# faircloth-lab/tapir

Hardware: AMD Instinct MI355X
Metric: alignment columns/sec (site-rate+PI) (higher is better)
Workload: dtype f64

## Files before the change

tapir_amd/csrc/pi_kernels.hpp:

```cpp
#pragma once
#include <hip/hip_runtime.h>
#include <cstdint>
#include "gtr_model.hpp"
#include "tree_program.hpp"
#include "quadpack_device.hpp"
#include "site_rate_params.hpp"
#include "pi_rate.hpp"
#include "tphip.h"

namespace tphip {

constexpr int kTimeTile = 16;
constexpr int kIvTile = 8;

struct ClassifyParams {
    const uint8_t* states;
    int64_t ncols_total;
    int32_t ntaxa;
    const LocusModel* models;
    const int64_t* locus_offsets;
    const int32_t* chunk_locus;
    const int32_t* chunk_index;
    double* rate;
    double* subst;
// ... 465 lines not shown
        }
        if ((bal[it] >> lane) & 1ull) {
            const int32_t col = (int32_t)(base + it * kCompactChunkBlock + threadIdx.x);
            const int before = woff + __popcll(bal[it] & below);
            if (kClasses) {
                const int erank = weoff + __popcll(bal_easy[it] & below);
                const int res = reserved_before(erank, reserve_q);
                const bool easy = (bal_easy[it] >> lane) & 1ull;
                if (easy && reserved_before((int64_t)erank + 1, reserve_q) != res) work_cols[lo + n_main + res] = col;
                else work_cols[lo + before - res] = col;
            } else {
                work_cols[lo + before] = col;
            }
        }
    }
}

__device__ __forceinline__ double wave_sum(double v) {
#pragma unroll
    for (int o = 32; o > 0; o >>= 1) v += __shfl_xor(v, o);
    return v;
}

__global__ __launch_bounds__(kPiBlock) void pi_partial_kernel(PiParams P) {
    __shared__ double red[kTimeTile][4];
    __shared__ double tile[kTimeTile][16 * 17];
    const int chunk = blockIdx.x;
    const int locus = P.chunk_locus[chunk];
    const int64_t lo = P.locus_offsets[locus], hi = P.locus_offsets[locus + 1];
    const int64_t base = lo + (int64_t)P.chunk_index[chunk] * kPiChunk;
    const int lane = threadIdx.x & 63, wave = threadIdx.x >> 6;
    double r[kPiColsPerThread];
    bool ok[kPiColsPerThread];
#pragma unroll
    for (int j = 0; j < kPiColsPerThread; ++j) {
        const int64_t col = base + j * kPiBlock + threadIdx.x;
        r[j] = (col < hi) ? finalize_rate(P, col) : __longlong_as_double(0x7ff8000000000000ll);
        ok[j] = isfinite(r[j]) && r[j] != 0.0;
    }
    {
        __shared__ double packed_rate[kPiChunk];
        __shared__ int wave_count[kPiBlock / 64];
        int c = 0;
#pragma unroll
        for (int j = 0; j < kPiColsPerThread; ++j) c += ok[j] ? 1 : 0;
        int inc = c;
#pragma unroll
        for (int o = 1; o < 64; o <<= 1) {
            const int up = __shfl_up(inc, o);
            if (lane >= o) inc += up;
        }
        if (lane == 63) wave_count[wave] = inc;
        __syncthreads();
        int pos = inc - c, total = 0;
#pragma unroll
        for (int w = 0; w < kPiBlock / 64; ++w) { pos += (w < wave) ? wave_count[w] : 0; total += wave_count[w]; }
#pragma unroll
        for (int j = 0; j < kPiColsPerThread; ++j) if (ok[j]) packed_rate[pos++] = r[j];
        __syncthreads();
#pragma unroll
        for (int j = 0; j < kPiColsPerThread; ++j) {
            const int idx = j * kPiBlock + (int)threadIdx.x;
            ok[j] = idx < total;
            r[j] = ok[j] ? packed_rate[idx] : __longlong_as_double(0x7ff8000000000000ll);
        }
    }
    const int Wp = P.T + 2 * P.n_i;
    double* out = P.partial + (size_t)chunk * Wp;
    for (int t0 = 0; t0 < P.T; t0 += kTimeTile) {
        double acc[kTimeTile];
#pragma unroll
        for (int i = 0; i < kTimeTile; ++i) acc[i] = 0.0;
#pragma unroll
        for (int j = 0; j < kPiColsPerThread; ++j) {
            if (!ok[j]) continue;
            const double c = 16.0 * (r[j] * r[j]);
            const double q = exp(-(4.0 * r[j]));
            double p = exp(-(4.0 * r[j] * (double)t0));
#pragma unroll
            for (int i = 0; i < kTimeTile; ++i) {
                acc[i] = fma(c * (double)(t0 + i), p, acc[i]);
                p *= q;
            }
        }
        {
            const int slot = (threadIdx.x >> 4) * 17 + (threadIdx.x & 15);
#pragma unroll
            for (int i = 0; i < kTimeTile; ++i) tile[i][slot] = acc[i];
        }
        __syncthreads();
        {
            const int i = threadIdx.x >> 4, seg = threadIdx.x & 15;
            const double* src = &tile[i][seg * 17];
            double sum = 0.0;
#pragma unroll
            for (int k = 0; k < 16; ++k) sum += src[k];
            sum += __shfl_xor(sum, 8);
            sum += __shfl_xor(sum, 4);
            sum += __shfl_xor(sum, 2);
            sum += __shfl_xor(sum, 1);
            if (seg == 0 && t0 + i < P.T) out[t0 + i] = sum;
        }
        __syncthreads();
    }
    for (int k0 = 0; k0 < P.n_i; k0 += kIvTile) {
        double si[kIvTile], se[kIvTile];
#pragma unroll
        for (int kk = 0; kk < kIvTile; ++kk) { si[kk] = 0.0; se[kk] = 0.0; }
#pragma unroll 1
        for (int j = 0; j < kPiColsPerThread; ++j) {
            if (!ok[j]) continue;
            GkFactors F;
            double have_h = -1.0;
#pragma unroll
            for (int kk = 0; kk < kIvTile; ++kk) {
                const int k = k0 + kk;
                if (k < P.n_i) {
                    const double a = (double)P.intervals[2 * k], b = (double)P.intervals[2 * k + 1];
                    double res, err = 0.0;
                    if (P.integ_mode == TPHIP_INTEG_QUADPACK) {
                        const double hl = 0.5 * (b - a);
                        if (4.0 * r[j] * hl < 30.0) {
                            if (hl != have_h) { gk_factors(r[j], hl, F); have_h = hl; }
                            quad_townsend_factored(a, b, r[j], F, res, err);
                        } else {
                            quad_townsend<false>(a, b, r[j], nullptr, res, err);
                        }
                    } else {
                        res = integral_closed(a, b, r[j]);
                    }
                    si[kk] += res;
                    se[kk] += err;
                }
            }
        }
#pragma unroll
        for (int kk = 0; kk < kIvTile; ++kk) {
            const int k = k0 + kk;
            if (k < P.n_i) {
                const double s1 = wave_sum(si[kk]), s2 = wave_sum(se[kk]);
                if (lane == 0) { red[2 * kk][wave] = s1; red[2 * kk + 1][wave] = s2; }
            }
        }
        __syncthreads();
        if (threadIdx.x < 2 * kIvTile && k0 + (int)(threadIdx.x >> 1) < P.n_i) {
            const int kk = threadIdx.x >> 1, which = threadIdx.x & 1;
            out[P.T + which * P.n_i + k0 + kk] =
                ((red[threadIdx.x][0] + red[threadIdx.x][1]) + red[threadIdx.x][2]) + red[threadIdx.x][3];
        }
        __syncthreads();
    }
}

constexpr int kPiReduceBlock = 64;
__global__ __launch_bounds__(kPiReduceBlock) void pi_reduce_kernel(const double* __restrict__ partial, const int64_t* __restrict__ locus_chunk_offsets,
                                 int32_t T, const int32_t* __restrict__ times, int32_t n_t, int32_t n_i,
                                 double* __restrict__ tables) {
    const int locus = blockIdx.x;
    const int64_t c0 = locus_chunk_offsets[locus], c1 = locus_chunk_offsets[locus + 1];
    const int Wp = T + 2 * n_i, W = T + n_t + 2 * n_i;
    double* row = tables + (size_t)locus * W;
    for (int w = threadIdx.x; w < Wp + n_t; w += blockDim.x) {
        const int src = (w < Wp) ? w : times[w - Wp];
        double s = 0.0;
        int64_t c = c0;
        for (; c + 8 <= c1; c += 8) {
            double v[8];
#pragma unroll
            for (int u = 0; u < 8; ++u) v[u] = partial[(size_t)(c + u) * Wp + src];
#pragma unroll
            for (int u = 0; u < 8; ++u) s += v[u];
        }
        for (; c < c1; ++c) s += partial[(size_t)c * Wp + src];
        const int dst = (w < T) ? w : (w < Wp ? w + n_t : T + (w - Wp));
        row[dst] = s;
    }
}

__global__ void corrected_rates_kernel(PiParams P, int64_t n, double* __restrict__ out) {
    const int64_t i = (int64_t)blockIdx.x * blockDim.x + threadIdx.x;
    if (i < n) out[i] = finalize_rate(P, i);
}

__global__ void townsend_dense_kernel(const double* __restrict__ rates, int64_t n, const double* __restrict__ times,
                                      int32_t n_times, double* __restrict__ out) {
    const int64_t i = (int64_t)blockIdx.x * blockDim.x + threadIdx.x;
    if (i >= n) return;
    const double r = rates[i];
    for (int k = 0; k < n_times; ++k) out[(size_t)k * n + i] = townsend_pi<false>(times[k], r, nullptr);
}

__global__ void quad_sites_kernel(const double* __restrict__ rates, int64_t n, double a, double b, int32_t integ_mode,
                                  double* __restrict__ integral, double* __restrict__ abserr) {
    const int64_t i = (int64_t)blockIdx.x * blockDim.x + threadIdx.x;
    if (i >= n) return;
    const double r = rates[i];
    double res = __longlong_as_double(0x7ff8000000000000ll), err = res;
    if (isfinite(r)) {
        err = 0.0;
        if (integ_mode == TPHIP_INTEG_QUADPACK) quad_townsend<false>(a, b, r, nullptr, res, err);
        else res = integral_closed(a, b, r);
    }
    integral[i] = res;
    abserr[i] = err;
}

__global__ __launch_bounds__(256) void state_histogram_kernel(const uint8_t* __restrict__ states, int64_t ncols_total,
                                                              int32_t ntaxa, const int64_t* __restrict__ locus_offsets,
                                                              unsigned long long* __restrict__ hist) {
    __shared__ unsigned int h[16];
    const int locus = blockIdx.x;
    const int64_t lo = locus_offsets[locus], hi = locus_offsets[locus + 1];
    if (threadIdx.x < 16) h[threadIdx.x] = 0;
    __syncthreads();
    unsigned int mine[16];
#pragma unroll
    for (int m = 0; m < 16; ++m) mine[m] = 0;
    for (int t = 0; t < ntaxa; ++t) {
        const uint8_t* row = states + (int64_t)t * ncols_total;
        for (int64_t c = lo + threadIdx.x; c < hi; c += blockDim.x) {
            unsigned m = row[c] & 15u;
            m = m ? m : 15u;
#pragma unroll
            for (int k = 0; k < 16; ++k) mine[k] += (m == (unsigned)k);
        }
    }
#pragma unroll
    for (int m = 0; m < 16; ++m) {
        unsigned v = mine[m];
        for (int o = 32; o > 0; o >>= 1) v += __shfl_xor(v, o);
        if ((threadIdx.x & 63) == 0) atomicAdd(&h[m], v);
    }
    __syncthreads();
    if (threadIdx.x < 16) hist[(size_t)locus * 16 + threadIdx.x] = h[threadIdx.x];
}

}
```

tapir_amd/csrc/site_launch_plan.hpp:

```cpp
#pragma once
#include <algorithm>
#include <cmath>
#include <cstddef>
#include <cstdint>
#include <cstdio>
#include <cstdlib>
#include <cstring>
#include <optional>
#include <utility>
#include <vector>

#include "launch_constants.hpp"
#include "tphip.h"

namespace tphip {

inline size_t site_lds_bytes(int depth) { return (kSiteLdsHeader + (size_t)depth * 12 * kSiteBlock) * sizeof(double); }
inline size_t mixed_lds_bytes(int depth) { return (kMixedLdsHeader + (size_t)depth * 12 * kSiteBlock) * sizeof(double); }

struct PlanKnobs {
    std::optional<long> site_chunk, site_waves, site_grid_mult;
    std::optional<char> site_spill, site_persistent, site_mixed, site_tail_order, site_share_work, compact_chunked, dedup;
    std::optional<double> site_first_fraction, site_reserve;
    std::optional<std::pair<double, double>> site_class_weights;
    std::optional<int> host_split;
};

constexpr const char* kPlanKnobNames[] = {
    "TPHIP_SITE_CHUNK", "TPHIP_SITE_SPILL", "TPHIP_SITE_PERSISTENT", "TPHIP_SITE_MIXED", "TPHIP_SITE_WAVES",
    "TPHIP_SITE_FIRST_FRACTION", "TPHIP_SITE_GRID_MULT", "TPHIP_SITE_TAIL_ORDER", "TPHIP_SITE_SHARE_WORK", "TPHIP_SITE_RESERVE",
    "TPHIP_SITE_CLASS_WEIGHTS", "TPHIP_COMPACT_CHUNKED", "TPHIP_DEDUP", "TPHIP_HOST_SPLIT"};

inline bool set_plan_knob(PlanKnobs* k, const char* name, const char* text) {
    const auto is = [name](const char* n) { return strcmp(name, n) == 0; };
    if (is("TPHIP_SITE_CHUNK")) k->site_chunk = atol(text);
    else if (is("TPHIP_SITE_SPILL")) k->site_spill = text[0];
    else if (is("TPHIP_SITE_PERSISTENT")) k->site_persistent = text[0];
    else if (is("TPHIP_SITE_MIXED")) k->site_mixed = text[0];
    else if (is("TPHIP_SITE_WAVES")) k->site_waves = atol(text);
    else if (is("TPHIP_SITE_FIRST_FRACTION")) k->site_first_fraction = atof(text);
    else if (is("TPHIP_SITE_GRID_MULT")) k->site_grid_mult = atol(text);
    else if (is("TPHIP_SITE_TAIL_ORDER")) k->site_tail_order = text[0];
    else if (is("TPHIP_SITE_SHARE_WORK")) k->site_share_work = text[0];
    else if (is("TPHIP_SITE_RESERVE")) k->site_reserve = atof(text);
    else if (is("TPHIP_SITE_CLASS_WEIGHTS")) {
        double a = 0, b = 0;
        if (sscanf(text, "%lf,%lf", &a, &b) == 2) k->site_class_weights = std::make_pair(a, b);
    }
    else if (is("TPHIP_COMPACT_CHUNKED")) k->compact_chunked = text[0];
    else if (is("TPHIP_DEDUP")) k->dedup = text[0];
    else if (is("TPHIP_HOST_SPLIT")) k->host_split = atoi(text);
    else return false;
    return true;
}

struct SiteShape {
    int64_t ncols = 0, nloci = 0, max_locus_cols = 0;
    int32_t ntaxa = 0;
    int32_t nwords = 0;
    int32_t stack_depth = 0;
    int32_t model = 0;
    int32_t ncat = 0;
    int32_t start_rule = 0;
    int32_t pattern_dedup = 0;
    int32_t T = 0, n_i = 0;
};

struct SiteLaunch {
    int32_t start_rule = 0;
    int32_t dedup_mode = 0;
    int32_t chunk_cols = kSiteBlock;
    int32_t waves = 0;
    int32_t persistent = 1;
    int32_t mixed_few_waves = 0;
    int64_t mixed_switch_cols = 0;
    int32_t mixed = 0;
    int32_t grid_mult = 1;
    int32_t lds_depth = 0;
    double first_fraction = 0.0;
    int32_t tail_order = 1;
    int32_t share_work = 0, reserve_q = 0, w_slow = 0, w_easy = 0;
    int32_t compact_chunked = 0;
};

inline int64_t site_grid(const SiteLaunch& s, int64_t n_site_chunks) {
    return s.mixed ? s.waves : s.persistent ? (int64_t)s.waves * s.grid_mult : n_site_chunks;
}

inline int32_t site_chunk_cols(const PlanKnobs& knobs) {
    int64_t cc = 512;
    if (knobs.site_chunk && *knobs.site_chunk >= kSiteBlock) cc = *knobs.site_chunk;
    return (int32_t)cc;
}

template <typename Occupancy>
SiteLaunch decide_site_launch(const SiteShape& shape, int num_cus, const PlanKnobs& knobs, Occupancy&& occupancy) {
    SiteLaunch s;
    const int64_t ncols = shape.ncols;
    const int nwords = shape.nwords, stack_depth = shape.stack_depth;
    s.start_rule = shape.start_rule == TPHIP_START_AUTO
                       ? ((shape.ntaxa >= kFirstStepMinTaxa || shape.ncat > 1) ? TPHIP_START_PARSIMONY : TPHIP_START_REFERENCE)
                       : shape.start_rule;
    s.chunk_cols = site_chunk_cols(knobs);
    int per_cu = occupancy(nwords <= 2 ? 2 : nwords <= 8 ? 8 : kStreamWords, site_lds_bytes(stack_depth));
    if (per_cu < 1) per_cu = 1;
    s.waves = per_cu * num_cus;
    s.lds_depth = stack_depth;
    {
        const int keep = (int)((160 * 1024 / 8 - kSiteLdsHeader * sizeof(double)) / (12 * kSiteBlock * sizeof(double)));
        bool want = nwords > 8 && stack_depth > keep && per_cu < 8;
        if (knobs.site_spill) want = (*knobs.site_spill == '1') && nwords > 8 && stack_depth > 1;
        if (want) {
            const int depth = std::max(1, std::min(keep, stack_depth - 1));
            const int per2 = occupancy(kStreamWordsSpill, site_lds_bytes(depth));
            if (per2 > per_cu && ncols / ((int64_t)per2 * num_cus) >= 1000) {
                s.lds_depth = depth;
                s.waves = per2 * num_cus;
            }
        }
    }
    s.persistent = (ncols / s.waves >= 1000) ? 1 : 0;
    if (knobs.site_persistent) s.persistent = (*knobs.site_persistent == '1');
    if (!s.persistent && s.lds_depth < stack_depth) {
        s.lds_depth = stack_depth;
        s.waves = per_cu * num_cus;
    }
    const bool mixed_fits = nwords <= 8 && ncols < ((int64_t)1 << kMixedColBits);
    s.mixed = (!s.persistent && mixed_fits) ? 1 : 0;
    if (knobs.site_mixed) s.mixed = (*knobs.site_mixed == '1') && mixed_fits;
    if (s.mixed) {
        int per3 = 0;
        const size_t lds3 = mixed_lds_bytes(stack_depth);
        const int64_t simds = 4 * (int64_t)num_cus;
        const double est_rounds = (double)ncols * (s.start_rule == TPHIP_START_REFERENCE ? 2.2 : 1.4) / (double)(kSiteBlock * simds);
        if (lds3 > 160 * 1024 || (per3 = occupancy(kMixedVariant + (nwords <= 2 ? 2 : 8), lds3)) < 1) s.mixed = 0;
        else if (est_rounds >= 28.0 && per3 < 8 && !knobs.site_mixed) s.mixed = 0;
        else {
            s.persistent = 0;
            const int64_t want = (per3 < 8) ? std::min<int64_t>(simds, (int64_t)per3 * num_cus) : 8 * (int64_t)num_cus;
            s.mixed_few_waves = (int32_t)std::min<int64_t>(simds, want);
            s.mixed_switch_cols = (int64_t)(24.0 * (double)(kSiteBlock * simds) / (s.start_rule == TPHIP_START_REFERENCE ? 3.7 : 2.4));
            s.waves = (int32_t)std::max<int64_t>(1, std::min<int64_t>(want, (ncols + kSiteBlock - 1) / kSiteBlock));
        }
    }
    if (knobs.site_waves && *knobs.site_waves >= 1) { s.waves = (int32_t)*knobs.site_waves; s.mixed_switch_cols = 0; }
    {
        const int64_t share = ncols / std::max(1, s.waves);
        const bool uneven = s.persistent && share >= 1500;
        s.grid_mult = uneven ? 3 : 1;
        const int64_t avg_locus = ncols / std::max<int64_t>(1, shape.nloci);
        s.first_fraction = !uneven ? 0.0 : (share >= 2 * avg_locus ? 0.9 : 0.8);
        if (uneven && s.lds_depth < stack_depth) s.first_fraction = 0.8;
        if (knobs.site_first_fraction) s.first_fraction = *knobs.site_first_fraction;
        if (knobs.site_grid_mult && *knobs.site_grid_mult >= 1 && *knobs.site_grid_mult <= 16) s.grid_mult = (int32_t)*knobs.site_grid_mult;
        if (knobs.site_tail_order) s.tail_order = (*knobs.site_tail_order != '0');
        double reserve = kDefaultReserve, w_slow = 2.9, w_easy = 2.04;
        s.share_work = (uneven && share < 2 * avg_locus) ? 1 : 0;
        if (knobs.site_share_work) s.share_work = (*knobs.site_share_work != '0');
        if (knobs.site_reserve) reserve = *knobs.site_reserve;
        if (knobs.site_class_weights) {
            const double a = knobs.site_class_weights->first, b = knobs.site_class_weights->second;
            if (a > 0 && b > 0 && a <= 16 && b <= 16) { w_slow = a; w_easy = b; }
        }
        if (!s.persistent || s.mixed || shape.max_locus_cols > ((int64_t)1 << 24)) s.share_work = 0;
        s.w_slow = std::max<int32_t>(1, (int32_t)lround(w_slow * (1 << kShareWeightShift)));
        s.w_easy = std::max<int32_t>(1, (int32_t)lround(w_easy * (1 << kShareWeightShift)));
        reserve = (s.share_work && s.grid_mult > 1) ? std::min(std::max(reserve, 0.0), 1.0) : 0.0;
        s.reserve_q = (int32_t)lround(reserve * (1 << kReserveShift));
    }
    s.compact_chunked = shape.max_locus_cols > 2048 ? 1 : 0;
    if (knobs.compact_chunked) s.compact_chunked = (*knobs.compact_chunked != '0');
    s.dedup_mode = shape.pattern_dedup;
    if (knobs.dedup)
        s.dedup_mode = (*knobs.dedup == '0') ? DEDUP_OFF : (*knobs.dedup == '1') ? DEDUP_ON : DEDUP_AUTO;
    if (s.dedup_mode == DEDUP_AUTO && ncols < kDedupAutoMinColumns) s.dedup_mode = DEDUP_OFF;
    return s;
}

inline int32_t host_split_groups(const PlanKnobs& knobs) {
    return knobs.host_split ? std::max(1, std::min(64, *knobs.host_split)) : 2;
}

struct ChunkTables {
    std::vector<int32_t> site_chunk_locus, site_chunk_index, pi_chunk_locus, pi_chunk_index;
    std::vector<int64_t> locus_pichunk_offsets;
};

inline ChunkTables build_chunk_tables(const int64_t* locus_offsets, int64_t nloci, int32_t chunk_cols) {
    ChunkTables t;
    t.locus_pichunk_offsets.assign((size_t)nloci + 1, 0);
    for (int64_t l = 0; l < nloci; ++l) {
        const int64_t S = locus_offsets[l + 1] - locus_offsets[l];
        const int64_t ns_max = std::max<int64_t>(1, (S + chunk_cols / 2) / chunk_cols);
        for (int64_t c = 0; c < ns_max && S > 0; ++c) { t.site_chunk_locus.push_back((int32_t)l); t.site_chunk_index.push_back((int32_t)c); }
        for (int64_t c = 0; c * kPiChunk < S; ++c) { t.pi_chunk_locus.push_back((int32_t)l); t.pi_chunk_index.push_back((int32_t)c); }
        t.locus_pichunk_offsets[l + 1] = (int64_t)t.pi_chunk_locus.size();
    }
    return t;
}

struct WorkspaceLayout {
    size_t work_cols = 0, work_cols2 = 0, work_count = 0, work_prefix = 0, slice_prefix = 0;
    size_t work_class = 0, work_wprefix = 0, part_prefix = 0, part_start = 0;
    size_t chunk_cnt = 0;
    size_t partial = 0, packed = 0;
    size_t hash = 0, dup_of = 0, tab_key = 0, tab_val = 0, dedup_on = 0;
    size_t spill = 0;
    size_t total = 0;
};

inline WorkspaceLayout layout_workspace(const SiteShape& shape, const SiteLaunch& s, int64_t n_pi_chunks) {
    WorkspaceLayout w;
    size_t off = 0;
    const auto take = [&off](size_t bytes) { const size_t at = off; off = (off + bytes + 255) / 256 * 256; return at; };
    const size_t ncols = (size_t)shape.ncols, nloci = (size_t)shape.nloci;
    w.work_cols = take(sizeof(int32_t) * ncols);
    if (!s.persistent || s.reserve_q > 0) w.work_cols2 = take(sizeof(int32_t) * ncols);
    w.work_count = take(sizeof(int32_t) * nloci);
    w.work_prefix = take(sizeof(int64_t) * (nloci + 1));
    w.slice_prefix = take(sizeof(int64_t) * (nloci + 1));
    w.work_class = take(sizeof(int32_t) * 2 * nloci);
    w.work_wprefix = take(sizeof(int64_t) * (nloci + 1));
    w.part_prefix = take(sizeof(int64_t) * 2 * (nloci + 1));
    w.part_start = take(sizeof(int64_t) * 2 * (nloci + 1));
    w.chunk_cnt = take(sizeof(int32_t) * 2 * (size_t)std::max<int64_t>(1, n_pi_chunks));
    w.partial = take(sizeof(double) * (size_t)n_pi_chunks * (size_t)(shape.T + 2 * shape.n_i));
    w.packed = take(sizeof(uint32_t) * (size_t)shape.nwords * ncols);
    if (s.dedup_mode != DEDUP_OFF) {
        w.hash = take(sizeof(uint64_t) * ncols);
        w.dup_of = take(sizeof(int32_t) * ncols);
        w.tab_key = take(sizeof(unsigned long long) * 2 * ncols);
        w.tab_val = take(sizeof(int32_t) * 2 * ncols);
        w.dedup_on = take(sizeof(int32_t) * nloci);
    }
    if (s.lds_depth < shape.stack_depth) {
        const size_t rows = (size_t)s.waves * (size_t)s.grid_mult * (size_t)(shape.stack_depth - s.lds_depth);
        w.spill = take(rows * 12 * kSiteBlock * sizeof(double));
    }
    w.total = off + 256;
    return w;
}

}
```

tapir_amd/csrc/tphip.hip:

```cpp
#include <hip/hip_runtime.h>

#include <algorithm>
#include <cmath>
#include <cstddef>
#include <cstdio>
#include <cstdlib>
#include <cstring>
#include <string>
#include <vector>

#include "gtr_model.hpp"
#include "gtr_setup_kernel.hpp"
#include "locus_lik_params.hpp"
#include "locus_value_params.hpp"
#include "pattern_kernels.hpp"
#include <hipcub/hipcub.hpp>
#include "pi_kernels.hpp"
#include "site_rate_params.hpp"
#include "tphip.h"
#include "tree_program.hpp"
#include "tphip_internal.hpp"

using namespace tphip;

// ... 561 lines not shown
    ClassifyParams C;
    C.states = d_states; C.ncols_total = p->ncols; C.ntaxa = p->ntaxa; C.models = p->d_models.p;
    C.locus_offsets = p->d_offsets.p; C.chunk_locus = p->d_pi_chunk_locus.p; C.chunk_index = p->d_pi_chunk_index.p;
    C.rate = d_rate; C.subst = d_subst; C.lnl = d_lnl; C.flag = d_flag; C.nres = d_nres;
    C.chrono_length = p->prog.chrono_length;
    C.steps = (const int2*)p->d_cls_steps.p; C.tail_pops = p->prog.cls_tail_pops; C.max_pops = p->prog.cls_max_pops;
    C.packed = (uint32_t*)((char*)ws + p->ws.packed);
    C.start_scale = (p->site.start_rule == TPHIP_START_REFERENCE) ? 0.0 : 1.0;
    const bool dedup = p->site.dedup_mode != DEDUP_OFF && p->n_pi_chunks > 0;
    C.hash = dedup ? (uint64_t*)((char*)ws + p->ws.hash) : nullptr;
    DedupParams D;
    if (dedup) {
        D.locus_offsets = p->d_offsets.p; D.chunk_locus = p->d_pi_chunk_locus.p; D.chunk_index = p->d_pi_chunk_index.p;
        D.hash = C.hash; D.packed = C.packed; D.nwords = p->nwords; D.ncols_total = p->ncols; D.flag = d_flag;
        D.dup_of = (int32_t*)((char*)ws + p->ws.dup_of);
        D.tab_key = (unsigned long long*)((char*)ws + p->ws.tab_key); D.tab_val = (int32_t*)((char*)ws + p->ws.tab_val);
        D.on = (int32_t*)((char*)ws + p->ws.dedup_on); D.mode = p->site.dedup_mode;
        D.rate = d_rate; D.subst = d_subst; D.lnl = d_lnl;
    }
    if (p->n_pi_chunks > 0) {
        classify_kernel<<<dim3((unsigned)p->n_pi_chunks), dim3(kPiBlock), 0, st>>>(C);
        if (dedup) {
            if (p->max_locus_cols > 2048) dedup_estimate_kernel<1024><<<dim3((unsigned)p->nloci), dim3(1024), 0, st>>>(D);
            else dedup_estimate_kernel<256><<<dim3((unsigned)p->nloci), dim3(256), 0, st>>>(D);
            dedup_insert_kernel<<<dim3((unsigned)p->n_pi_chunks), dim3(256), 0, st>>>(D);
            dedup_resolve_kernel<<<dim3((unsigned)p->n_pi_chunks), dim3(256), 0, st>>>(D);
        }
        if (p->site.share_work) {
            int32_t* work_class = (int32_t*)((char*)ws + p->ws.work_class);
            if (p->site.compact_chunked) {
                launch_compact_chunked(p, d_flag, d_lnl, work_cols, work_count, work_class, ws, st);
            } else {
                int32_t* scratch = p->site.reserve_q > 0 ? (int32_t*)((char*)ws + p->ws.work_cols2) : nullptr;
                if (p->max_locus_cols > 2048) compact_classes_kernel<1024><<<dim3((unsigned)p->nloci), dim3(1024), 0, st>>>(d_flag, p->d_offsets.p, work_cols, work_count, d_lnl, p->site.reserve_q, scratch, work_class);
                else compact_classes_kernel<256><<<dim3((unsigned)p->nloci), dim3(256), 0, st>>>(d_flag, p->d_offsets.p, work_cols, work_count, d_lnl, p->site.reserve_q, scratch, work_class);
            }
            ScanClasses SC;
            SC.cls = work_class; SC.reserve_q = p->site.reserve_q; SC.w_slow = p->site.w_slow; SC.w_easy = p->site.w_easy;
            SC.locus_offsets = p->d_offsets.p;
            SC.wprefix = (int64_t*)((char*)ws + p->ws.work_wprefix); SC.part_prefix = (int64_t*)((char*)ws + p->ws.part_prefix);
            SC.part_start = (int64_t*)((char*)ws + p->ws.part_start);
            HIP_TRY(launch_scan_counts_kernel(st, work_count, p->nloci, p->site.chunk_cols, (int64_t*)((char*)ws + p->ws.work_prefix),
                                              (int64_t*)((char*)ws + p->ws.slice_prefix), &SC));
        } else {
            if (p->site.compact_chunked) launch_compact_chunked(p, d_flag, nullptr, work_cols, work_count, nullptr, ws, st);
            else if (p->max_locus_cols > 2048) compact_kernel<1024><<<dim3((unsigned)p->nloci), dim3(1024), 0, st>>>(d_flag, p->d_offsets.p, work_cols, work_count);
            else compact_kernel<256><<<dim3((unsigned)p->nloci), dim3(256), 0, st>>>(d_flag, p->d_offsets.p, work_cols, work_count);
            HIP_TRY(launch_scan_counts_kernel(st, work_count, p->nloci, p->site.chunk_cols, (int64_t*)((char*)ws + p->ws.work_prefix),
                                              (int64_t*)((char*)ws + p->ws.slice_prefix), nullptr));
        }
    }
    HIP_TRY(hipMemsetAsync(p->d_evals.p, 0, 8 * sizeof(unsigned long long), st));
    SiteParams S;
    S.states = d_states; S.ncols_total = p->ncols; S.models = p->d_models.p; S.ops = p->d_ops.p;
    S.nops = (int32_t)p->prog.ops.size(); S.stack_depth = p->prog.stack_depth; S.chrono_length = p->prog.chrono_length;
    S.locus_offsets = p->d_offsets.p; S.chunk_locus = p->d_site_chunk_locus.p; S.chunk_index = p->d_site_chunk_index.p;
    S.chunk_cols = p->site.chunk_cols;
    S.packed = (const uint32_t*)((char*)ws + p->ws.packed); S.nwords = p->nwords;
    S.work_cols = work_cols; S.work_count = work_count;
    S.work_cols2 = (!p->site.persistent && p->ws.work_cols2) ? (int32_t*)((char*)ws + p->ws.work_cols2) : nullptr;
    S.work_prefix = (const int64_t*)((char*)ws + p->ws.work_prefix); S.nloci = p->nloci;
    S.slice_prefix = (const int64_t*)((char*)ws + p->ws.slice_prefix);
    S.rate = d_rate; S.subst = d_subst; S.lnl = d_lnl; S.flag = d_flag; S.eval_counter = p->d_evals.p;
    const bool spill = p->site.lds_depth < p->prog.stack_depth;
    S.lds_depth = p->site.lds_depth;
    S.spill = spill ? (double*)((char*)ws + p->ws.spill) : nullptr;
    S.persistent = (p->site.persistent || p->site.mixed) ? 1 : 0;
    S.first_round = p->site.waves;
    S.mixed_few_waves = p->site.mixed_few_waves; S.mixed_switch_cols = p->site.mixed_switch_cols;
    S.tail_order = (p->site.persistent && !p->site.mixed && p->site.tail_order) ? 1 : 0;
    S.first_fraction = (p->site.first_fraction > 0.0) ? p->site.first_fraction : 1.0 / (double)p->site.grid_mult;
    S.share_work = p->site.share_work;
    S.main_shares = (p->site.reserve_q > 0) ? p->site.waves : p->site.waves * p->site.grid_mult;
    S.work_wprefix = (const int64_t*)((char*)ws + p->ws.work_wprefix); S.part_prefix = (const int64_t*)((char*)ws + p->ws.part_prefix);
    S.part_start = (const int64_t*)((char*)ws + p->ws.part_start);
    S.ncat = p->ncat; S.cat = p->d_cat.p;
    if (slot >= 0) HIP_TRY(hipEventRecord(p->ev[4 * slot + 0], st));
    if (p->n_site_chunks > 0) {
        const bool mixed = p->site.mixed;
        const dim3 grid((unsigned)site_grid(p->site, p->n_site_chunks));
        S.ops = p->d_fused_ops.p;
        S.nops = (int32_t)p->prog.fused_ops.size();
        const int variant = p->nwords <= 2 ? 2 : p->nwords <= 8 ? 8 : (spill ? kStreamWordsSpill : kStreamWords);
        if (mixed) {
            S.first_fraction = 1.0;
            HIP_TRY(launch_site_rate_kernel(kMixedVariant + variant, p->model, grid, mixed_lds_bytes(p->prog.stack_depth), st, S));
        } else
            HIP_TRY(launch_site_rate_kernel(variant, p->model, grid, site_lds_bytes(p->site.lds_depth), st, S));
    }
    if (slot >= 0) HIP_TRY(hipEventRecord(p->ev[4 * slot + 1], st));
    if (dedup) dedup_scatter_kernel<<<dim3((unsigned)p->n_pi_chunks), dim3(256), 0, st>>>(D);
    HIP_TRY(hipGetLastError());
    return TPHIP_OK;
}

__global__ __launch_bounds__(256) void eb_start_scale_kernel(const int64_t* __restrict__ locus_offsets, const uint8_t* __restrict__ flag,
                                                            const double* __restrict__ start_log, double chrono_length,
                                                            double* __restrict__ start) {
    __shared__ double red[256];
    const int locus = blockIdx.x;
    const int64_t lo = locus_offsets[locus], hi = locus_offsets[locus + 1];
    double sum = 0.0;
    for (int64_t c = lo + threadIdx.x; c < hi; c += 256)
        if (flag[c] == TPHIP_FLAG_OK) sum += exp(start_log[c]);
    red[threadIdx.x] = sum;
    __syncthreads();
    for (int o = 128; o > 0; o >>= 1) {
        if ((int)threadIdx.x < o) red[threadIdx.x] += red[threadIdx.x + o];
        __syncthreads();
    }
    if (threadIdx.x == 0) start[locus] = (red[0] > 0.0 && hi > lo) ? red[0] / (double)(hi - lo) : 1.0 / chrono_length;
}

int tphip_internal_eb_prepare(tphip_plan* p, const uint8_t* d_states, const EbPrep* B, int32_t use_patterns, double* d_start,
                              void* stream) {
    hipStream_t st = (hipStream_t)stream;
    if (p->n_pi_chunks <= 0) return TPHIP_OK;
    ClassifyParams C;
    C.states = d_states; C.ncols_total = p->ncols; C.ntaxa = p->ntaxa; C.models = p->d_models.p;
    C.locus_offsets = p->d_offsets.p; C.chunk_locus = p->d_pi_chunk_locus.p; C.chunk_index = p->d_pi_chunk_index.p;
    C.rate = B->scratch[0]; C.subst = B->scratch[1]; C.lnl = B->scratch[2]; C.flag = B->flag; C.nres = B->nres;
    C.chrono_length = p->prog.chrono_length;
    C.steps = (const int2*)p->d_cls_steps.p; C.tail_pops = p->prog.cls_tail_pops; C.max_pops = p->prog.cls_max_pops;
    C.packed = B->packed;
    C.start_scale = 1.0;
    C.hash = use_patterns ? B->hash : nullptr;
    classify_kernel<<<dim3((unsigned)p->n_pi_chunks), dim3(kPiBlock), 0, st>>>(C);
    if (d_start)
        eb_start_scale_kernel<<<dim3((unsigned)p->nloci), dim3(256), 0, st>>>(p->d_offsets.p, B->flag, B->scratch[0],
                                                                             p->prog.chrono_length, d_start);
    HIP_TRY(hipMemsetAsync(B->flag, TPHIP_FLAG_OK, (size_t)p->ncols, st));
    HIP_TRY(hipMemsetAsync(B->dup_of, 0xff, sizeof(int32_t) * (size_t)p->ncols, st));
    if (use_patterns) {
        DedupParams D;
        D.locus_offsets = p->d_offsets.p; D.chunk_locus = p->d_pi_chunk_locus.p; D.chunk_index = p->d_pi_chunk_index.p;
        D.hash = B->hash; D.packed = B->packed; D.nwords = p->nwords; D.ncols_total = p->ncols; D.flag = B->flag;
        D.dup_of = B->dup_of; D.tab_key = B->tab_key; D.tab_val = B->tab_val; D.on = B->on; D.mode = DEDUP_ON;
        D.rate = nullptr; D.subst = nullptr; D.lnl = nullptr;
        if (p->max_locus_cols > 2048) dedup_estimate_kernel<1024><<<dim3((unsigned)p->nloci), dim3(1024), 0, st>>>(D);
        else dedup_estimate_kernel<256><<<dim3((unsigned)p->nloci), dim3(256), 0, st>>>(D);
        dedup_insert_kernel<<<dim3((unsigned)p->n_pi_chunks), dim3(256), 0, st>>>(D);
        dedup_resolve_kernel<<<dim3((unsigned)p->n_pi_chunks), dim3(256), 0, st>>>(D);
        if (p->max_locus_cols > 2048) compact_kernel<1024><<<dim3((unsigned)p->nloci), dim3(1024), 0, st>>>(B->flag, p->d_offsets.p, B->work_cols, B->work_count);
        else compact_kernel<256><<<dim3((unsigned)p->nloci), dim3(256), 0, st>>>(B->flag, p->d_offsets.p, B->work_cols, B->work_count);
    }
    HIP_TRY(hipGetLastError());
    return TPHIP_OK;
}

static int launch_pi_tables(tphip_plan* p, const double* d_rates, const int32_t* d_nres, double* d_tables, void* ws,
                            hipStream_t st, int slot) {
    PiParams Q = pi_params(p, d_rates, d_nres, ws);
    if (slot >= 0) HIP_TRY(hipEventRecord(p->ev[4 * slot + 2], st));
    if (p->n_pi_chunks > 0) pi_partial_kernel<<<dim3((unsigned)p->n_pi_chunks), dim3(kPiBlock), 0, st>>>(Q);
    pi_reduce_kernel<<<dim3((unsigned)p->nloci), dim3(kPiReduceBlock), 0, st>>>(Q.partial, p->d_locus_pichunk_offsets.p, p->T,
                                                                   p->d_times.p, p->n_t, p->n_i, d_tables);
    if (slot >= 0) HIP_TRY(hipEventRecord(p->ev[4 * slot + 3], st));
    HIP_TRY(hipGetLastError());
    return TPHIP_OK;
}

static int take_slot(tphip_plan* p) {
    if (!p->profile) return -1;
    if (p->ev_used >= kProfileRing) {
        if (profile_drain(p)) return -1;
    }
    return p->ev_used++;
}

int tphip_run_dev(tphip_plan* p, const uint8_t* d_states, double* d_rate, double* d_subst, double* d_lnl, uint8_t* d_flag,
                  int32_t* d_nres, double* d_tables, void* ws, size_t ws_bytes, void* stream) {
    if (!p) return fail(TPHIP_ERR_INVALID, "null plan");
    if (!d_states || !d_rate || !d_subst || !d_lnl || !d_flag || !d_nres || !d_tables || !ws)
        return fail(TPHIP_ERR_INVALID, "null device pointer");
    if (ws_bytes < p->ws.total) return fail(TPHIP_ERR_WORKSPACE, "workspace smaller than tphip_plan_workspace_bytes()");
    HIP_TRY(hipSetDevice(p->device));
    hipStream_t st = (hipStream_t)stream;
    int slot = take_slot(p);
    int rc = launch_site_rates(p, d_states, d_rate, d_subst, d_lnl, d_flag, d_nres, ws, st, slot);
    if (rc) return rc;
    return launch_pi_tables(p, d_rate, d_nres, d_tables, ws, st, slot);
}

int tphip_site_rates_dev(tphip_plan* p, const uint8_t* d_states, double* d_rate, double* d_subst, double* d_lnl,
                         uint8_t* d_flag, int32_t* d_nres, void* ws, size_t ws_bytes, void* stream) {
    if (!p) return fail(TPHIP_ERR_INVALID, "null plan");
    if (!d_states || !d_rate || !d_subst || !d_lnl || !d_flag || !d_nres || !ws)
        return fail(TPHIP_ERR_INVALID, "null device pointer");
    if (ws_bytes < p->ws.total) return fail(TPHIP_ERR_WORKSPACE, "workspace smaller than tphip_plan_workspace_bytes()");
    HIP_TRY(hipSetDevice(p->device));
    int slot = take_slot(p);
    int rc = launch_site_rates(p, d_states, d_rate, d_subst, d_lnl, d_flag, d_nres, ws, (hipStream_t)stream, slot);
    if (rc == 0 && slot >= 0) {
        HIP_TRY(hipEventRecord(p->ev[4 * slot + 2], (hipStream_t)stream));
        HIP_TRY(hipEventRecord(p->ev[4 * slot + 3], (hipStream_t)stream));
    }
    return rc;
}

int tphip_pi_tables_dev(tphip_plan* p, const double* d_rates, const int32_t* d_nres, double* d_tables, void* ws,
                        size_t ws_bytes, void* stream) {
    if (!p) return fail(TPHIP_ERR_INVALID, "null plan");
    if (!d_rates || !d_tables || !ws) return fail(TPHIP_ERR_INVALID, "null device pointer");
    if (ws_bytes < p->ws.total) return fail(TPHIP_ERR_WORKSPACE, "workspace smaller than tphip_plan_workspace_bytes()");
    HIP_TRY(hipSetDevice(p->device));
    int slot = take_slot(p);
    if (slot >= 0) {
        HIP_TRY(hipEventRecord(p->ev[4 * slot + 0], (hipStream_t)stream));
        HIP_TRY(hipEventRecord(p->ev[4 * slot + 1], (hipStream_t)stream));
    }
    return launch_pi_tables(p, d_rates, d_nres, d_tables, ws, (hipStream_t)stream, slot);
}

static PiParams pi_params(const tphip_plan* p, const double* d_rates, const int32_t* d_nres, void* ws) {
    PiParams Q;
    Q.rates = d_rates; Q.nres = d_nres; Q.locus_offsets = p->d_offsets.p;
    Q.chunk_locus = p->d_pi_chunk_locus.p; Q.chunk_index = p->d_pi_chunk_index.p;
    Q.T = p->T; Q.intervals = p->d_intervals.p; Q.n_i = p->n_i; Q.integ_mode = p->integ_mode;
    Q.correction = p->correction; Q.threshold = p->threshold;
    Q.round_scale = (p->round_decimals >= 0) ? std::pow(10.0, (double)p->round_decimals) : 0.0;
    Q.partial = ws ? (double*)((char*)ws + p->ws.partial) : nullptr;
    return Q;
}

int tphip_corrected_rates_dev(tphip_plan* p, const double* d_rates, const int32_t* d_nres, double* d_out, void* stream) {
    if (!p) return fail(TPHIP_ERR_INVALID, "null plan");
    if (p->ncols && (!d_rates || !d_out)) return fail(TPHIP_ERR_INVALID, "null device pointer");
    HIP_TRY(hipSetDevice(p->device));
    if (p->ncols) {
        corrected_rates_kernel<<<dim3((unsigned)((p->ncols + 255) / 256)), dim3(256), 0, (hipStream_t)stream>>>(
            pi_params(p, d_rates, d_nres, nullptr), p->ncols, d_out);
        HIP_TRY(hipGetLastError());
    }
    return TPHIP_OK;
}

int tphip_corrected_rates(tphip_plan* p, const double* rates, const int32_t* nres, double* out) {
    if (!p) return fail(TPHIP_ERR_INVALID, "null plan");
    if (p->ncols == 0) return TPHIP_OK;
    if (!rates || !out) return fail(TPHIP_ERR_INVALID, "null host pointer");
    HIP_TRY(hipSetDevice(p->device));
    Scratch S;
    const size_t n = (size_t)p->ncols;
    double* d_r = S.get<double>(n);
    double* d_o = S.get<double>(n);
    int32_t* d_n = nres ? S.get<int32_t>(n) : nullptr;
    if (!d_r || !d_o || (nres && !d_n)) return fail(TPHIP_ERR_HIP, "hipMalloc failed");
    HIP_TRY(hipMemcpy(d_r, rates, sizeof(double) * n, hipMemcpyHostToDevice));
    if (nres) HIP_TRY(hipMemcpy(d_n, nres, sizeof(int32_t) * n, hipMemcpyHostToDevice));
    int rc = tphip_corrected_rates_dev(p, d_r, d_n, d_o, nullptr);
    if (rc) return rc;
    HIP_TRY(hipMemcpy(out, d_o, sizeof(double) * n, hipMemcpyDeviceToHost));
    return TPHIP_OK;
}

int tphip_townsend_pi_dense_dev(int32_t device, const double* d_rates, int64_t n, const double* d_times, int32_t n_times,
                                double* d_out, void* stream) {
    if (tphip_device_count() <= 0) return fail(TPHIP_ERR_NO_DEVICE, "no HIP device visible: libtphip has no CPU path");
    if (n < 0 || n_times < 0 || (n && n_times && (!d_rates || !d_out || !d_times))) return fail(TPHIP_ERR_INVALID, "bad arguments");
    HIP_TRY(hipSetDevice(device));
    if (n && n_times) {
        townsend_dense_kernel<<<dim3((unsigned)((n + 255) / 256)), dim3(256), 0, (hipStream_t)stream>>>(d_rates, n, d_times,
                                                                                                    n_times, d_out);
        HIP_TRY(hipGetLastError());
    }
    return TPHIP_OK;
}

int tphip_quad_townsend_dev(int32_t device, const double* d_rates, int64_t n, double a, double b, int32_t integ_mode,
                            double* d_integral, double* d_abserr, void* stream) {
    if (tphip_device_count() <= 0) return fail(TPHIP_ERR_NO_DEVICE, "no HIP device visible: libtphip has no CPU path");
    if (n < 0 || (n && (!d_rates || !d_integral || !d_abserr))) return fail(TPHIP_ERR_INVALID, "bad arguments");
    if (!(a < b)) return fail(TPHIP_ERR_INVALID, "Start time is sooner than end time in an interval");
    if (integ_mode != TPHIP_INTEG_QUADPACK && integ_mode != TPHIP_INTEG_CLOSED) return fail(TPHIP_ERR_INVALID, "unknown integ_mode");
    HIP_TRY(hipSetDevice(device));
    if (n) {
        quad_sites_kernel<<<dim3((unsigned)((n + 127) / 128)), dim3(128), 0, (hipStream_t)stream>>>(d_rates, n, a, b, integ_mode,
                                                                                                d_integral, d_abserr);
        HIP_TRY(hipGetLastError());
    }
    return TPHIP_OK;
}

static int lik_nsplit(const tphip_plan* p, int64_t ncand, int block) {
    const int64_t target = (int64_t)p->num_cus * 8;
    int64_t ns = (target + ncand - 1) / std::max<int64_t>(ncand, 1);
    const int64_t max_blocks = std::max<int64_t>(1, (p->max_locus_cols + block - 1) / block);
    ns = std::min(ns, max_blocks);
    return (int)std::max<int64_t>(1, std::min<int64_t>(ns, 4096));
}

static int grow(void** ptr, size_t& have, size_t need) {
    if (need <= have && *ptr) return TPHIP_OK;
    if (*ptr) { HIP_TRY(hipFree(*ptr)); *ptr = nullptr; have = 0; }
    HIP_TRY(hipMalloc(ptr, need ? need : 1));
    have = need;
    return TPHIP_OK;
}

int tphip_locus_loglik_dev(tphip_plan* p, const uint8_t* d_states, int64_t ncand, const int32_t* d_cand_locus,
                           const double* d_cand_exch, const double* d_blen_vecs, const int32_t* d_cand_vec,
                           const double* d_cand_scale, const int32_t* d_cand_pidx, const double* d_cand_pfac, double* d_out,
                           void* stream) {
    if (!p) return fail(TPHIP_ERR_INVALID, "null plan");
    if (ncand < 0 || (ncand && (!d_states || !d_cand_locus || !d_cand_exch || !d_blen_vecs || !d_cand_vec || !d_cand_scale ||
                                !d_cand_pidx || !d_cand_pfac || !d_out)))
        return fail(TPHIP_ERR_INVALID, "null device pointer");
// ... 822 lines not shown
```

Measured before the change: 784.0 million.

## Split PI partial kernel into separate net-PI and interval kernels for long loci

```diff
diff --git a/tapir_amd/csrc/pi_kernels.hpp b/tapir_amd/csrc/pi_kernels.hpp
--- a/tapir_amd/csrc/pi_kernels.hpp
+++ b/tapir_amd/csrc/pi_kernels.hpp
@@ -641,6 +641,175 @@
     }
 }
 
+
+__device__ __forceinline__ void pi_pack_chunk(const PiParams& P, int64_t base, int64_t hi, double* packed_rate, double* r, bool* ok) {
+    __shared__ int wave_count[kPiBlock / 64];
+    const int lane = threadIdx.x & 63, wave = threadIdx.x >> 6;
+#pragma unroll
+    for (int j = 0; j < kPiColsPerThread; ++j) {
+        const int64_t col = base + j * kPiBlock + threadIdx.x;
+        r[j] = (col < hi) ? finalize_rate(P, col) : __longlong_as_double(0x7ff8000000000000ll);
+        ok[j] = isfinite(r[j]) && r[j] != 0.0;
+    }
+    int c = 0;
+#pragma unroll
+    for (int j = 0; j < kPiColsPerThread; ++j) c += ok[j] ? 1 : 0;
+    int inc = c;
+#pragma unroll
+    for (int o = 1; o < 64; o <<= 1) {
+        const int up = __shfl_up(inc, o);
+        if (lane >= o) inc += up;
+    }
+    if (lane == 63) wave_count[wave] = inc;
+    __syncthreads();
+    int pos = inc - c, total = 0;
+#pragma unroll
+    for (int w = 0; w < kPiBlock / 64; ++w) { pos += (w < wave) ? wave_count[w] : 0; total += wave_count[w]; }
+#pragma unroll
+    for (int j = 0; j < kPiColsPerThread; ++j) if (ok[j]) packed_rate[pos++] = r[j];
+    __syncthreads();
+#pragma unroll
+    for (int j = 0; j < kPiColsPerThread; ++j) {
+        const int idx = j * kPiBlock + (int)threadIdx.x;
+        ok[j] = idx < total;
+        r[j] = ok[j] ? packed_rate[idx] : __longlong_as_double(0x7ff8000000000000ll);
+    }
+}
+
+__global__ __launch_bounds__(kPiBlock, 4) void pi_net_kernel(PiParams P) {
+    __shared__ double tile[kTimeTile][16 * 17];
+    static_assert(kTimeTile * 16 * 17 >= kPiChunk, "the transpose buffer holds a chunk's packed rates");
+    const int chunk = blockIdx.x;
+    const int locus = P.chunk_locus[chunk];
+    const int64_t lo = P.locus_offsets[locus], hi = P.locus_offsets[locus + 1];
+    const int64_t base = lo + (int64_t)P.chunk_index[chunk] * kPiChunk;
+    double r[kPiColsPerThread];
+    bool ok[kPiColsPerThread];
+    pi_pack_chunk(P, base, hi, &tile[0][0], r, ok);
+    __syncthreads();
+    double* out = P.partial + (size_t)chunk * (P.T + 2 * P.n_i);
+    for (int t0 = 0; t0 < P.T; t0 += kTimeTile) {
+        double acc[kTimeTile], t[kTimeTile];
+#pragma unroll
+        for (int i = 0; i < kTimeTile; ++i) { acc[i] = 0.0; t[i] = (double)(t0 + i); }
+#pragma unroll
+        for (int j = 0; j < kPiColsPerThread; ++j) {
+            if (!ok[j]) continue;
+            const double c = 16.0 * (r[j] * r[j]);
+            const double q = exp(-(4.0 * r[j]));
+            double p = exp(-(4.0 * r[j] * (double)t0));
+#pragma unroll
+            for (int i = 0; i < kTimeTile; ++i) {
+                acc[i] = fma(c * t[i], p, acc[i]);
+                p *= q;
+            }
+        }
+        {
+            const int slot = (threadIdx.x >> 4) * 17 + (threadIdx.x & 15);
+#pragma unroll
+            for (int i = 0; i < kTimeTile; ++i) tile[i][slot] = acc[i];
+        }
+        __syncthreads();
+        {
+            const int i = threadIdx.x >> 4, seg = threadIdx.x & 15;
+            const double* src = &tile[i][seg * 17];
+            double sum = 0.0;
+#pragma unroll
+            for (int k = 0; k < 16; ++k) sum += src[k];
+            sum += __shfl_xor(sum, 8);
+            sum += __shfl_xor(sum, 4);
+            sum += __shfl_xor(sum, 2);
+            sum += __shfl_xor(sum, 1);
+            if (seg == 0 && t0 + i < P.T) out[t0 + i] = sum;
+        }
+        __syncthreads();
+    }
+}
+
+struct QuadResult { double result, abserr; };
+__device__ __noinline__ QuadResult quad_townsend_generic(double a, double b, double rate) {
+    QuadResult o;
+    o.abserr = 0.0;
+    quad_townsend<false>(a, b, rate, nullptr, o.result, o.abserr);
+    return o;
+}
+
+constexpr int kIvSplitTile = 4;
+__global__ __launch_bounds__(kPiBlock, 2) void pi_interval_kernel(PiParams P) {
+    __shared__ double red[2 * kIvSplitTile][4];
+    __shared__ double packed_rate[kPiChunk];
+    const int chunk = blockIdx.x;
+    const int locus = P.chunk_locus[chunk];
+    const int64_t lo = P.locus_offsets[locus], hi = P.locus_offsets[locus + 1];
+    const int64_t base = lo + (int64_t)P.chunk_index[chunk] * kPiChunk;
+    const int lane = threadIdx.x & 63, wave = threadIdx.x >> 6;
+    int n_ok = 0;
+    {
+        double r[kPiColsPerThread];
+        bool ok[kPiColsPerThread];
+        pi_pack_chunk(P, base, hi, packed_rate, r, ok);
+#pragma unroll
+        for (int j = 0; j < kPiColsPerThread; ++j) n_ok += ok[j] ? 1 : 0;
+    }
+    double* out = P.partial + (size_t)chunk * (P.T + 2 * P.n_i);
+    for (int k0 = 0; k0 < P.n_i; k0 += kIvSplitTile) {
+        int a[kIvSplitTile], b[kIvSplitTile];
+#pragma unroll
+        for (int kk = 0; kk < kIvSplitTile; ++kk) {
+            const int k = (k0 + kk < P.n_i) ? k0 + kk : P.n_i - 1;
+            a[kk] = __builtin_amdgcn_readfirstlane(P.intervals[2 * k]);
+            b[kk] = __builtin_amdgcn_readfirstlane(P.intervals[2 * k + 1]);
+        }
+        double si[kIvSplitTile], se[kIvSplitTile];
+#pragma unroll
+        for (int kk = 0; kk < kIvSplitTile; ++kk) { si[kk] = 0.0; se[kk] = 0.0; }
+#pragma unroll 1
+        for (int j = 0; j < n_ok; ++j) {
+            const double rj = packed_rate[j * kPiBlock + (int)threadIdx.x];
+            GkFactors F;
+            double have_h = -1.0;
+#pragma unroll
+            for (int kk = 0; kk < kIvSplitTile; ++kk) {
+                if (k0 + kk < P.n_i) {
+                    int ai = a[kk], bi = b[kk];
+                    asm volatile("" : "+s"(ai), "+s"(bi));
+                    const double aj = (double)ai, bj = (double)bi;
+                    double res, err = 0.0;
+                    if (P.integ_mode == TPHIP_INTEG_QUADPACK) {
+                        const double hl = 0.5 * (bj - aj);
+                        if (4.0 * rj * hl < 30.0) {
+                            if (hl != have_h) { gk_factors(rj, hl, F); have_h = hl; }
+                            quad_townsend_factored(aj, bj, rj, F, res, err);
+                        } else {
+                            const QuadResult g = quad_townsend_generic(aj, bj, rj);
+                            res = g.result;
+                            err = g.abserr;
+                        }
+                    } else {
+                        res = integral_closed(aj, bj, rj);
+                    }
+                    si[kk] += res;
+                    se[kk] += err;
+                }
+            }
+        }
+#pragma unroll
+        for (int kk = 0; kk < kIvSplitTile; ++kk) {
+            if (k0 + kk < P.n_i) {
+                const double s1 = wave_sum(si[kk]), s2 = wave_sum(se[kk]);
+                if (lane == 0) { red[2 * kk][wave] = s1; red[2 * kk + 1][wave] = s2; }
+            }
+        }
+        __syncthreads();
+        if (threadIdx.x < 2 * kIvSplitTile && k0 + (int)(threadIdx.x >> 1) < P.n_i) {
+            const int kk = threadIdx.x >> 1, which = threadIdx.x & 1;
+            out[P.T + which * P.n_i + k0 + kk] =
+                ((red[threadIdx.x][0] + red[threadIdx.x][1]) + red[threadIdx.x][2]) + red[threadIdx.x][3];
+        }
+        __syncthreads();
+    }
+}
+
 constexpr int kPiReduceBlock = 64;
 __global__ __launch_bounds__(kPiReduceBlock) void pi_reduce_kernel(const double* __restrict__ partial, const int64_t* __restrict__ locus_chunk_offsets,
                                  int32_t T, const int32_t* __restrict__ times, int32_t n_t, int32_t n_i,
diff --git a/tapir_amd/csrc/site_launch_plan.hpp b/tapir_amd/csrc/site_launch_plan.hpp
--- a/tapir_amd/csrc/site_launch_plan.hpp
+++ b/tapir_amd/csrc/site_launch_plan.hpp
@@ -20,7 +20,7 @@
 
 struct PlanKnobs {
     std::optional<long> site_chunk, site_waves, site_grid_mult;
-    std::optional<char> site_spill, site_persistent, site_mixed, site_tail_order, site_share_work, compact_chunked, dedup;
+    std::optional<char> site_spill, site_persistent, site_mixed, site_tail_order, site_share_work, compact_chunked, pi_split, dedup;
     std::optional<double> site_first_fraction, site_reserve;
     std::optional<std::pair<double, double>> site_class_weights;
     std::optional<int> host_split;
@@ -29,7 +29,7 @@
 constexpr const char* kPlanKnobNames[] = {
     "TPHIP_SITE_CHUNK", "TPHIP_SITE_SPILL", "TPHIP_SITE_PERSISTENT", "TPHIP_SITE_MIXED", "TPHIP_SITE_WAVES",
     "TPHIP_SITE_FIRST_FRACTION", "TPHIP_SITE_GRID_MULT", "TPHIP_SITE_TAIL_ORDER", "TPHIP_SITE_SHARE_WORK", "TPHIP_SITE_RESERVE",
-    "TPHIP_SITE_CLASS_WEIGHTS", "TPHIP_COMPACT_CHUNKED", "TPHIP_DEDUP", "TPHIP_HOST_SPLIT"};
+    "TPHIP_SITE_CLASS_WEIGHTS", "TPHIP_COMPACT_CHUNKED", "TPHIP_PI_SPLIT", "TPHIP_DEDUP", "TPHIP_HOST_SPLIT"};
 
 inline bool set_plan_knob(PlanKnobs* k, const char* name, const char* text) {
     const auto is = [name](const char* n) { return strcmp(name, n) == 0; };
@@ -48,6 +48,7 @@
         if (sscanf(text, "%lf,%lf", &a, &b) == 2) k->site_class_weights = std::make_pair(a, b);
     }
     else if (is("TPHIP_COMPACT_CHUNKED")) k->compact_chunked = text[0];
+    else if (is("TPHIP_PI_SPLIT")) k->pi_split = text[0];
     else if (is("TPHIP_DEDUP")) k->dedup = text[0];
     else if (is("TPHIP_HOST_SPLIT")) k->host_split = atoi(text);
     else return false;
@@ -81,6 +82,7 @@
     int32_t tail_order = 1;
     int32_t share_work = 0, reserve_q = 0, w_slow = 0, w_easy = 0;
     int32_t compact_chunked = 0;
+    int32_t pi_split = 0;
 };
 
 inline int64_t site_grid(const SiteLaunch& s, int64_t n_site_chunks) {
@@ -170,6 +172,8 @@
     }
     s.compact_chunked = shape.max_locus_cols > 2048 ? 1 : 0;
     if (knobs.compact_chunked) s.compact_chunked = (*knobs.compact_chunked != '0');
+    s.pi_split = shape.max_locus_cols > 2048 ? 1 : 0;
+    if (knobs.pi_split) s.pi_split = (*knobs.pi_split != '0');
     s.dedup_mode = shape.pattern_dedup;
     if (knobs.dedup)
         s.dedup_mode = (*knobs.dedup == '0') ? DEDUP_OFF : (*knobs.dedup == '1') ? DEDUP_ON : DEDUP_AUTO;
diff --git a/tapir_amd/csrc/tphip.hip b/tapir_amd/csrc/tphip.hip
--- a/tapir_amd/csrc/tphip.hip
+++ b/tapir_amd/csrc/tphip.hip
@@ -737,7 +737,15 @@
                             hipStream_t st, int slot) {
     PiParams Q = pi_params(p, d_rates, d_nres, ws);
     if (slot >= 0) HIP_TRY(hipEventRecord(p->ev[4 * slot + 2], st));
-    if (p->n_pi_chunks > 0) pi_partial_kernel<<<dim3((unsigned)p->n_pi_chunks), dim3(kPiBlock), 0, st>>>(Q);
+    if (p->n_pi_chunks > 0) {
+        const dim3 grid((unsigned)p->n_pi_chunks), block(kPiBlock);
+        if (p->site.pi_split) {
+            pi_net_kernel<<<grid, block, 0, st>>>(Q);
+            if (p->n_i > 0) pi_interval_kernel<<<grid, block, 0, st>>>(Q);
+        } else {
+            pi_partial_kernel<<<grid, block, 0, st>>>(Q);
+        }
+    }
     pi_reduce_kernel<<<dim3((unsigned)p->nloci), dim3(kPiReduceBlock), 0, st>>>(Q.partial, p->d_locus_pichunk_offsets.p, p->T,
                                                                    p->d_times.p, p->n_t, p->n_i, d_tables);
     if (slot >= 0) HIP_TRY(hipEventRecord(p->ev[4 * slot + 3], st));
```

New measurement: 793.3 million, median of 6. 1.2% higher.
